# daniestevez/gr4-packet-modem

Hardware: AMD Instinct MI355X
Metric: RX Msamples/s (syncword-detect + RRC chain) (higher is better)
Workload: dtype f32; 1 GPU; configs[1]: 1 channel/GPU, full RX front end (SyncwordDetection 9 bins FFT 2048 + tag gate + CFC + 32-arm RRC SymbolFilter + wipe-off + Costas) on resident burst+AWGN stream; channels_per_gpu=1, freq_bins=9, parallelism=channel-per-gpu x1, input=generated on each GPU, pipelined_streams=4, pipeline_driver=native (gr4pm_packet_receiver), windows=2, correlator_lookahead=2

## Files before the change

### gr4-packet-modem_amd/_abi.py

```python
import ctypes as C
import os

import numpy as np

_HERE = os.path.dirname(os.path.abspath(__file__))
LIB_PATH = os.environ.get("GR4PM_LIB") or os.path.join(_HERE, "libgr4pm_hip.so")

OK = 0
INSUFFICIENT_INPUT_ITEMS = 1
INSUFFICIENT_OUTPUT_ITEMS = 2
TAG_SYNCWORD = 1
TAG_OTHER = 2

TAG_DTYPE = np.dtype(
    [
        ("index", "<u8"),
        ("amplitude", "<f4"),
        ("phase", "<f4"),
        ("freq", "<f8"),
        ("freq_bin", "<i4"),
        ("noise_power", "<f4"),
        ("esn0_db", "<f4"),
        ("time_est", "<f4"),
        ("flags", "<i4"),
# ... 144 lines not shown
                ("pdu_symbols", C.c_void_p), ("n_pdu_symbols", C.c_size_t), ("symbol_pdus", C.c_void_p),
                ("n_symbol_pdus", C.c_size_t), ("symbol_pdu_resyncs", C.c_size_t)]


SYMBOL_PDU_DTYPE = np.dtype([("offset", "<u8"), ("length", "<u8"), ("kind", "<i4"), ("first", "<i4"), ("last", "<i4"),
                             ("pad", "<i4")])
SYMBOL_PDU_FN = C.CFUNCTYPE(None, C.c_void_p, C.c_int, C.c_void_p, C.c_size_t)


class PfbArbParams(C.Structure):
    _fields_ = [("rate", C.c_double), ("rate_is_double", C.c_int), ("taps", C.c_void_p),
                ("n_taps", C.c_size_t), ("filter_size", C.c_size_t), ("stream", C.c_void_p)]


class NoiseSourceParams(C.Structure):
    _fields_ = [("item_kind", C.c_int), ("noise_type", C.c_int), ("amplitude", C.c_float), ("seed", C.c_uint64),
                ("max_items", C.c_size_t), ("stream", C.c_void_p)]


EXPORTS = [
    "gr4pm_last_error", "gr4pm_version", "gr4pm_device_count", "gr4pm_set_deferred_sync", "gr4pm_sincosf", "gr4pm_costas_phase_wrap",
    "gr4pm_packet_receiver_set_symbol_pdu_callback",
    "gr4pm_packet_receiver_publish_symbol_pdus",
    "gr4pm_zmq_pub_create",
    "gr4pm_zmq_pub_destroy",
    "gr4pm_zmq_pub_send",
    "gr4pm_zmq_pub_port",
    "gr4pm_zmq_pub_subscribers",
    "gr4pm_zmq_pub_dropped",
    "gr4pm_syncword_detection_create", "gr4pm_syncword_detection_destroy",
    "gr4pm_syncword_detection_reset", "gr4pm_syncword_detection_syncword_samples_size",
    "gr4pm_syncword_detection_self_corr", "gr4pm_syncword_detection_items_consumed", "gr4pm_syncword_detection_scan_counts",
    "gr4pm_syncword_detection_process", "gr4pm_syncword_detection_last_zpow",
    "gr4pm_syncword_detection_correlate_only",
    "gr4pm_syncword_detection_hint_next", "gr4pm_syncword_detection_announce",
    "gr4pm_syncword_detection_filter_create", "gr4pm_syncword_detection_filter_destroy",
    "gr4pm_syncword_detection_filter_reset", "gr4pm_syncword_detection_filter_process",
    "gr4pm_syncword_detection_filter_gate", "gr4pm_syncword_detection_filter_gate_resolve",
    "gr4pm_payload_metadata_insert_resolve",
    "gr4pm_rotator_create", "gr4pm_rotator_destroy", "gr4pm_rotator_reset", "gr4pm_rotator_process",
    "gr4pm_costas_loop_create", "gr4pm_costas_loop_destroy", "gr4pm_costas_loop_reset",
    "gr4pm_costas_loop_coeffs", "gr4pm_costas_loop_set", "gr4pm_costas_loop_process",
    "gr4pm_syncword_wipeoff_create", "gr4pm_syncword_wipeoff_destroy", "gr4pm_syncword_wipeoff_reset",
    "gr4pm_syncword_wipeoff_process",
    "gr4pm_interp_fir_create", "gr4pm_interp_fir_destroy", "gr4pm_interp_fir_reset",
    "gr4pm_interp_fir_process",
    "gr4pm_symbol_filter_create", "gr4pm_symbol_filter_destroy", "gr4pm_symbol_filter_reset",
    "gr4pm_symbol_filter_process", "gr4pm_cfc_symbol_filter_process",
    "gr4pm_cfc_symbol_filter_plan", "gr4pm_cfc_symbol_filter_run",
    "gr4pm_cfc_symbol_filter_plan_channels", "gr4pm_cfc_symbol_filter_run_channel",
    "gr4pm_cfc_symbol_filter_run_channels", "gr4pm_syncword_wipeoff_process_channels",
    "gr4pm_multichannel_receiver_set_input_in_place", "gr4pm_costas_loop_process_ragged", "gr4pm_costas_loop_set_small_footprint",
    "gr4pm_pfb_arb_resampler_create", "gr4pm_pfb_arb_resampler_destroy", "gr4pm_pfb_arb_resampler_reset",
    "gr4pm_pfb_arb_resampler_process",
    "gr4pm_firdes_root_raised_cosine",
    "gr4pm_payload_metadata_insert_create", "gr4pm_payload_metadata_insert_destroy",
    "gr4pm_payload_metadata_insert_reset", "gr4pm_payload_metadata_insert_process",
    "gr4pm_costas_loop_process_packets",
    "gr4pm_syncword_remove_create", "gr4pm_syncword_remove_destroy", "gr4pm_syncword_remove_reset",
    "gr4pm_syncword_remove_process",
    "gr4pm_constellation_llr_decoder_create", "gr4pm_constellation_llr_decoder_destroy",
    "gr4pm_constellation_llr_decoder_process",
    "gr4pm_additive_scrambler_create", "gr4pm_additive_scrambler_destroy", "gr4pm_additive_scrambler_reset",
    "gr4pm_additive_scrambler_process",
    "gr4pm_header_payload_split_create", "gr4pm_header_payload_split_destroy",
    "gr4pm_header_payload_split_reset", "gr4pm_header_payload_split_process", "gr4pm_header_payload_split_process_c64",
# ... 25 lines not shown
    if _lib is not None:
        return _lib
    if not os.path.exists(LIB_PATH):
        raise ImportError(
            f"{LIB_PATH} is missing: build it with `python -c 'import __graft_entry__ as g; g.build()'` "
            "(hipcc --offload-arch=gfx950). There is no CPU fallback.")
    try:
        import torch
    except ImportError:
        pass
    L = C.CDLL(LIB_PATH)
    vp, sz, szp = C.c_void_p, C.c_size_t, C.POINTER(C.c_size_t)
    L.gr4pm_last_error.restype = C.c_char_p
    L.gr4pm_version.restype = C.c_char_p
    L.gr4pm_device_count.restype = C.c_int
    if hasattr(L, "gr4pm_test_fail_allocations"):
        L.gr4pm_test_fail_allocations.argtypes = [C.c_long, C.c_long]
        L.gr4pm_test_fail_allocations.restype = None
        L.gr4pm_test_allocation_count.restype = C.c_ulonglong
    L.gr4pm_syncword_detection_create.argtypes = [C.POINTER(SyncwordDetectionParams), C.POINTER(vp)]
    L.gr4pm_syncword_detection_destroy.argtypes = [vp]
    L.gr4pm_syncword_detection_destroy.restype = None
    L.gr4pm_syncword_detection_reset.argtypes = [vp]
    L.gr4pm_syncword_detection_syncword_samples_size.argtypes = [vp]
    L.gr4pm_syncword_detection_syncword_samples_size.restype = sz
    L.gr4pm_syncword_detection_self_corr.argtypes = [vp]
    L.gr4pm_syncword_detection_self_corr.restype = C.c_float
    L.gr4pm_syncword_detection_items_consumed.argtypes = [vp]
    L.gr4pm_syncword_detection_items_consumed.restype = C.c_uint64
    L.gr4pm_syncword_detection_scan_counts.argtypes = [vp, sz, C.POINTER(C.c_uint64), C.POINTER(C.c_uint64)]
    L.gr4pm_syncword_detection_scan_counts.restype = None
    L.gr4pm_syncword_detection_process.argtypes = [vp, vp, sz, sz, vp, sz, szp, vp, sz, vp]
    L.gr4pm_syncword_detection_last_zpow.argtypes = [vp, vp, sz]
    L.gr4pm_syncword_detection_correlate_only.argtypes = [vp, vp, sz, sz]
    L.gr4pm_syncword_detection_hint_next.argtypes = [vp, vp, sz, sz]
    L.gr4pm_syncword_detection_announce.argtypes = [vp, vp, sz, sz]
    L.gr4pm_syncword_detection_filter_create.argtypes = [C.POINTER(SdfParams), C.POINTER(vp)]
    L.gr4pm_syncword_detection_filter_destroy.argtypes = [vp]
    L.gr4pm_syncword_detection_filter_destroy.restype = None
    L.gr4pm_syncword_detection_filter_reset.argtypes = [vp]
    L.gr4pm_syncword_detection_filter_process.argtypes = [vp, vp, sz, vp, sz, C.c_int, vp, sz, sz, szp, szp, szp,
                                                          C.POINTER(C.c_int)]
    L.gr4pm_syncword_detection_filter_gate.argtypes = [vp, vp, sz, vp, sz, C.c_int, vp, szp]
    L.gr4pm_rotator_create.argtypes = [C.POINTER(RotatorParams), C.POINTER(vp)]
    L.gr4pm_rotator_destroy.argtypes = [vp]
    L.gr4pm_rotator_destroy.restype = None
    L.gr4pm_rotator_reset.argtypes = [vp]
    L.gr4pm_rotator_process.argtypes = [vp, vp, sz, sz, vp, vp, vp, sz]
    L.gr4pm_costas_loop_create.argtypes = [C.POINTER(CostasParams), C.POINTER(vp)]
    L.gr4pm_costas_loop_destroy.argtypes = [vp]
    L.gr4pm_costas_loop_destroy.restype = None
    L.gr4pm_costas_loop_reset.argtypes = [vp]
    L.gr4pm_costas_loop_coeffs.argtypes = [vp, C.POINTER(C.c_float), C.POINTER(C.c_float)]
    L.gr4pm_costas_loop_coeffs.restype = None
    L.gr4pm_costas_loop_set.argtypes = [vp, C.c_double, C.c_int]
    L.gr4pm_costas_loop_process.argtypes = [vp, vp, sz, sz, vp, vp, vp, sz]
    L.gr4pm_syncword_wipeoff_create.argtypes = [C.POINTER(WipeoffParams), C.POINTER(vp)]
    L.gr4pm_syncword_wipeoff_destroy.argtypes = [vp]
    L.gr4pm_syncword_wipeoff_destroy.restype = None
    L.gr4pm_syncword_wipeoff_reset.argtypes = [vp]
    L.gr4pm_syncword_wipeoff_process.argtypes = [vp, vp, sz, vp, vp, sz]
    L.gr4pm_syncword_wipeoff_process_channels.argtypes = [vp, sz, vp, sz, vp, vp, vp]
    L.gr4pm_cfc_symbol_filter_run_channels.argtypes = [vp, C.c_int, vp, sz, vp, sz, sz, vp, sz, vp, vp, vp, sz, vp, vp, vp, sz, sz]
    L.gr4pm_multichannel_receiver_set_input_in_place.argtypes = [vp, C.c_int]
    L.gr4pm_interp_fir_create.argtypes = [C.POINTER(InterpFirParams), C.POINTER(vp)]
    L.gr4pm_interp_fir_destroy.argtypes = [vp]
# ... 118 lines not shown
```

### gr4-packet-modem_amd/blocks.py

```python
import ctypes as C
import os

import numpy as np

from . import _abi
from ._abi import PACKET_TAG_DTYPE, TAG_DTYPE, TAG_OTHER, TAG_SYNCWORD, Gr4pmError, check, lib

CONSTELLATIONS = {"PILOT": 0, "BPSK": 1, "QPSK": 2}


def _torch():
    import torch
    return torch


def _stream_handle():
    torch = _torch()
    if not torch.cuda.is_available():
        raise Gr4pmError("no HIP device: the gr4pm blocks have no CPU fallback")
    return C.c_void_p(torch.cuda.current_stream().cuda_stream)


def _release(name, h):
    try:
# ... 159 lines not shown
            nx = _dev_c64(next_x)
            nx2 = nx.reshape(1, -1) if nx.dim() == 1 else nx
            assert nx2.shape[0] == self.n_channels
            check(lib().gr4pm_syncword_detection_hint_next(self._h, nx2.data_ptr(), nx2.stride(0), nx2.shape[1]),
                  "SyncwordDetection.hint_next")
        out = torch.empty_like(x2) if want_output else None
        n_done = C.c_size_t(0)
        tags = np.zeros((self.n_channels, tags_cap), dtype=TAG_DTYPE)
        n_tags = (C.c_size_t * self.n_channels)()
        st = lib().gr4pm_syncword_detection_process(
            self._h, x2.data_ptr(), x2.stride(0), n_in, out.data_ptr() if want_output else None,
            out.stride(0) if want_output else 0, C.byref(n_done), _np_ptr(tags), tags_cap, n_tags)
        check(st, "SyncwordDetection.processBulk")
        n = n_done.value
        tag_list = [tags[c, : n_tags[c]].copy() for c in range(self.n_channels)]
        if want_output:
            out = out[:, :n]
            if x.dim() == 1:
                out = out[0]
        if x.dim() == 1:
            tag_list = tag_list[0]
        return st, out, tag_list, n

    def correlate_only(self, x):
        x2 = x.reshape(1, -1) if x.dim() == 1 else x
        check(lib().gr4pm_syncword_detection_correlate_only(self._h, x2.data_ptr(), x2.stride(0), x2.shape[1]),
              "correlate_only")

    def last_zpow(self, n_done):
        torch = _torch()
        z = torch.empty((self.n_channels, n_done), dtype=torch.float32, device="cuda")
        check(lib().gr4pm_syncword_detection_last_zpow(self._h, z.data_ptr(), z.stride(0)), "last_zpow")
        return z

    def _destroy(self):
        if getattr(self, "_h", None):
            _release("gr4pm_syncword_detection_destroy", self._h)
            self._h = None

    def __del__(self):
        try:
            self._destroy()
        except Exception:
            pass


class SyncwordDetectionFilter:

    def __init__(self, samples_per_symbol=4, syncword_size=64, header_size=128):
        self.samples_per_symbol, self.syncword_size, self.header_size = samples_per_symbol, syncword_size, header_size
        p = _abi.SdfParams(samples_per_symbol, syncword_size, header_size, _stream_handle())
        self._h = C.c_void_p()
        check(lib().gr4pm_syncword_detection_filter_create(C.byref(p), C.byref(self._h)), "SyncwordDetectionFilter")

    def start(self):
        check(lib().gr4pm_syncword_detection_filter_reset(self._h), "start")

    def process_bulk(self, x, out, head_tag_flags=0, headers=(), n_ignored=0):
        x = _dev_c64(x)
        msgs = (_abi.HeaderMsg * max(len(headers), 1))()
        for i, hm in enumerate(headers):
            msgs[i].packet_length = 0 if hm is None else hm
            msgs[i].invalid_header = 1 if hm is None else 0
        c, hc, ic, tf = C.c_size_t(0), C.c_size_t(0), C.c_size_t(0), C.c_int(0)
        check(lib().gr4pm_syncword_detection_filter_process(
            self._h, x.data_ptr(), x.numel(), out.data_ptr(), out.numel(), head_tag_flags, msgs, len(headers),
# ... 1558 lines not shown
```

### gr4-packet-modem_amd/csrc/syncword_detection.hip

```cpp
#include <algorithm>
#include <chrono>
#include <cmath>
#include <complex>
#include <cstdint>
#include <deque>
#include <string>
#include <vector>

#include "common.hpp"
#include "fft2048_wave.hpp"
#include "fft2048_pair.hpp"
#include "fft2048_w64.hpp"

#ifndef GR4PM_ABL
#define GR4PM_ABL 0
#endif

namespace gr4pm {

namespace {

constexpr int kWavesPerWg = 4;
constexpr int kMaxBins = 64;
#ifndef GR4PM_TILE_W
#define GR4PM_TILE_W 32768
#endif
constexpr uint32_t kTileW = GR4PM_TILE_W;
constexpr int kAhead = 2, kSets = kAhead + 1, kCarry = kAhead + 2;

struct RawTag {
    uint64_t pos;
    float zx, zy;
    float zpow, left, right, prev, next, noise;
    int32_t bin_idx;
    int32_t pad;
};

__device__ __forceinline__ void wave_lds_sync()
{
    asm volatile("" ::: "memory");
    __builtin_amdgcn_wave_barrier();
    asm volatile("" ::: "memory");
}

__device__ __forceinline__ void fft1_wave(int lane, cf* r, cf* lds, const cf* tw1a, const cf* tw1b)
// ... 502 lines not shown
    }
#pragma unroll
    for (int q = (2 * TQ - 1) / 4 * 4; q < 2 * TQ - 1; ++q) acc += full[q] < thr ? 1u : 0u;
    acc += (at_or_before && prv[R] < thr) ? 1u : 0u;
    acc += (at_or_after && nxt[R] < thr) ? 1u : 0u;
    asm volatile("s_nop 1\n\t"
                 "v_add_u32_dpp %0, %0, %0 row_shr:1 row_mask:0xf bank_mask:0xf bound_ctrl:0\n\t"
                 "s_nop 1\n\t"
                 "v_add_u32_dpp %0, %0, %0 row_shr:2 row_mask:0xf bank_mask:0xf bound_ctrl:0\n\t"
                 "s_nop 1\n\t"
                 "v_add_u32_dpp %0, %0, %0 row_shr:4 row_mask:0xf bank_mask:0xf bound_ctrl:0\n\t"
                 "s_nop 1\n\t"
                 "v_add_u32_dpp %0, %0, %0 row_shr:8 row_mask:0xf bank_mask:0xf bound_ctrl:0\n\t"
                 "s_nop 1\n\t"
                 "v_add_u32_dpp %0, %0, %0 row_bcast:15 row_mask:0xa bank_mask:0xf\n\t"
                 "s_nop 1\n\t"
                 "v_add_u32_dpp %0, %0, %0 row_bcast:31 row_mask:0xc bank_mask:0xf"
                 : "+v"(acc));
    const uint32_t below = static_cast<uint32_t>(__builtin_amdgcn_readlane(static_cast<int>(acc), 63));
    return 2u * below >= 2u * T + 1u;
}
template <int TQ, int R>
__device__ __forceinline__ bool median_dispatch(int r, const float* prv, const float* cur, const float* nxt, int lp, int lane,
                                                float power_threshold)
{
    if constexpr (R >= TQ) {
        return false;
    } else {
        if (r == R) return median_in_registers<TQ, R>(prv, cur, nxt, lp, lane, power_threshold);
        return median_dispatch<TQ, R + 1>(r, prv, cur, nxt, lp, lane, power_threshold);
    }
}

template <int TQ, bool MEDIAN>
__global__ __launch_bounds__(64) void k_candidates_wave(const float* __restrict__ zbase, size_t z_stride, uint32_t cnt,
                                                        uint32_t n_words, uint32_t chain,
                                                        unsigned long long* __restrict__ bitmap, size_t bm_stride,
                                                        unsigned long long* __restrict__ passmap,
                                                        unsigned long long* __restrict__ defermap, float power_threshold)
{
    constexpr uint32_t T = TQ * 64;
    const int lane = threadIdx.x, rl = 63 - lane;
    const float* z = zbase + static_cast<size_t>(blockIdx.y) * z_stride;
    unsigned long long* bmp = bitmap + static_cast<size_t>(blockIdx.y) * bm_stride;
    unsigned long long* pmp = MEDIAN ? passmap + 2 * static_cast<size_t>(blockIdx.y) * bm_stride : nullptr;
    (void)defermap;
    constexpr uint32_t kTestsPerBlock = 8;
    const uint32_t avail = cnt + T;
    const uint32_t n_blk = (n_words + TQ - 1) / TQ;
    const uint32_t b0 = blockIdx.x * chain;
    if (b0 >= n_blk) return;
    const uint32_t b1 = min(b0 + chain, n_blk);
    auto load = [&](uint32_t b, float* v) {
        if ((b + 1) * T <= avail) {
            const char* zb = reinterpret_cast<const char*>(z + static_cast<size_t>(b) * T);
            const uint32_t voff = 4u * static_cast<uint32_t>(rl);
#pragma unroll
            for (int r = 0; r < TQ; ++r)
                v[r] = *reinterpret_cast<const float*>(zb + static_cast<size_t>(voff) + 256 * r);
            return;
        }
#pragma unroll
        for (int r = 0; r < TQ; ++r) {
            const uint32_t g = b * T + 64u * r + rl;
            v[r] = g < avail ? z[g] : -INFINITY;
        }
    };
    auto scans = [&](const float* v, int* rowmax) {
        float t[TQ];
#pragma unroll
        for (int r = 0; r < TQ; ++r) t[r] = v[r];
        if constexpr (TQ % 4 == 0) {
#pragma unroll
            for (int r = 0; r < TQ; r += 4) wave_prefix_max4(t[r], t[r + 1], t[r + 2], t[r + 3]);
        } else {
#pragma unroll
            for (int r = 0; r < TQ; ++r) t[r] = wave_prefix_max(t[r]);
        }
#pragma unroll
        for (int r = 0; r < TQ; ++r) rowmax[r] = fkey(__builtin_amdgcn_readlane(__builtin_bit_cast(int, t[r]), 63));
    };
    const int ninf = fkey(__builtin_bit_cast(int, -INFINITY));
    float cur[TQ], nxt[TQ], prv[MEDIAN ? TQ : 1];
    int rowmax[TQ];
    load(b0, cur);
    if (MEDIAN) {
#pragma unroll
        for (int r = 0; r < TQ; ++r) {
            const long long g = static_cast<long long>(b0) * T - static_cast<long long>(T) + 64 * r + rl;
            prv[r] = g < static_cast<long long>(avail) ? z[g] : -INFINITY;
        }
    }
    scans(cur, rowmax);
    unsigned long long before_mine = 0;
    for (uint32_t b = b0; b < b1; ++b) {
        load(b + 1, nxt);
        int nrowmax[TQ], before[TQ];
        scans(nxt, nrowmax);
        before[0] = ninf;
#pragma unroll
        for (int r = 1; r < TQ; ++r) before[r] = max(before[r - 1], nrowmax[r - 1]);
        unsigned long long mine = 0;
        int after = ninf;
#pragma unroll
        for (int r = TQ - 1; r >= 0; --r) {
            const int U = max(after, before[r]);
            unsigned long long word = 0;
            if (rowmax[r] >= U) {
                const float fwd = __shfl(nxt[r], rl);
                const float pr = __shfl(wave_prefix_max(fwd), rl);
                const float sfx = wave_prefix_max(cur[r]);
                const float m = fmaxf(fmaxf(wave_prev(sfx), __builtin_bit_cast(float, fkey(U))), pr);
                const uint32_t pos = b * T + 64u * r + rl;
                word = __brevll(__ballot(pos < cnt && cur[r] >= m));
            }
            if (lane == r) mine = word;
            after = max(after, rowmax[r]);
        }
        unsigned long long mine_pass = 0, mine_defer = 0;
        if (MEDIAN) {
            unsigned long long rows = __ballot(mine != 0);
            uint32_t tests_left = kTestsPerBlock;
            int prev_pos = -1;
            const bool have_before = b != b0;
            while (rows) {
                const int r = __ffsll(static_cast<long long>(rows)) - 1;
                rows &= rows - 1;
                const unsigned long long word =
                    (static_cast<unsigned long long>(static_cast<uint32_t>(__builtin_amdgcn_readlane(static_cast<int>(mine >> 32), r))) << 32) |
                    static_cast<uint32_t>(__builtin_amdgcn_readlane(static_cast<int>(mine), r));
// ... 9 lines not shown
                    const int o = 64 * r + bit;
                    bool visitable = true;
                    if (prev_pos >= 0) {
                        visitable = false;
                        if (have_before) {
                            const int lo = prev_pos, hi = o - 1, rlo = lo >> 6, rhi = hi >> 6;
                            unsigned long long mask = ~0ull;
                            if (lane == rlo) mask &= ~0ull << (lo & 63);
                            if (lane == rhi) mask &= ~0ull >> (63 - (hi & 63));
                            visitable = __ballot(lane >= rlo && lane <= rhi && (before_mine & mask) != 0) != 0;
                        }
                    }
                    prev_pos = o;
                    if (visitable && tests_left != 0) {
                        --tests_left;
                        if (median_dispatch<TQ, 0>(r, prv, cur, nxt, 63 - bit, lane, power_threshold)) passed |= 1ull << bit;
                    } else {
                        deferred |= 1ull << bit;
                    }
                }
                if (lane == r) {
                    mine_pass = passed;
                    mine_defer = deferred;
                }
            }
            before_mine = mine;
        }
        const uint32_t w = b * TQ + lane;
        if (lane < TQ && w < n_words) {
            bmp[w] = mine;
            if (MEDIAN)
                reinterpret_cast<ulonglong2*>(pmp)[w] = make_ulonglong2(mine_pass, mine_defer);
        }
#pragma unroll
        for (int r = 0; r < TQ; ++r) {
            if (MEDIAN) prv[r] = cur[r];
            cur[r] = nxt[r];
            rowmax[r] = nrowmax[r];
        }
    }
}


__device__ __forceinline__ uint32_t next_candidate(const unsigned long long* bm, uint32_t r, uint32_t hi)
{
    if (r >= hi) return hi;
    uint32_t w = r >> 6;
    unsigned long long word = bm[w] & (~0ull << (r & 63));
    const uint32_t wlast = (hi - 1) >> 6;
    while (true) {
        if (word) {
            const uint32_t p = (w << 6) + static_cast<uint32_t>(__ffsll(static_cast<long long>(word)) - 1);
            return p < hi ? p : hi;
        }
        if (w == wlast) return hi;
        word = bm[++w];
    }
}

constexpr int kTileChunks = static_cast<int>(kTileW / 4096);
static_assert(kTileW % 4096 == 0 && kTileChunks >= 1 && kTileChunks <= 16, "tile = whole 4096-item chunks");
struct TileBits {
    unsigned long long w[kTileChunks];
    uint32_t lo;
    __device__ __forceinline__ void load(const unsigned long long* bm, uint32_t lo_, uint32_t hi, int lane)
    {
        lo = __builtin_amdgcn_readfirstlane(lo_);
        const uint32_t w0 = lo >> 6, wlast = (hi - 1) >> 6;
#pragma unroll
        for (int k = 0; k < kTileChunks; ++k) {
            const uint32_t wi = w0 + 64u * k + lane;
// ... 935 lines not shown
        for (size_t i = 0; i < n; i += len) {
            for (size_t k = 0; k < len / 2; ++k) {
                const double ang = -2.0 * M_PI * static_cast<double>(k) / static_cast<double>(len);
                const std::complex<double> w(std::cos(ang), std::sin(ang));
                const auto u = a[i + k], v = a[i + k + len / 2] * w;
                a[i + k] = u + v;
                a[i + k + len / 2] = u - v;
            }
        }
    }
}

}
}

using namespace gr4pm;

struct gr4pm_syncword_detection {
    size_t fft_size, sps, n_channels, max_items;
    int min_bin, max_bin, n_bins;
    uint64_t T;
    float power_threshold;
    hipStream_t stream;
    size_t L, S, hist;
    float self_corr;
    uint32_t xc, zc;
    size_t z_stride, bm_stride, table_stride;
    uint32_t noise_off = 0;
    uint32_t max_tiles, det_cap, rec_cap;
    DevBuf<float4> tmpl;
    DevBuf<cf> tw;
    bool lds_candidates = false;
    bool separate_median = false;
    bool w64_no_prune = false;
    int corr_kind = 0;
    DevBuf<float4> tmpl64, tT64;
    DevBuf<cf> td;
    DevBuf<cf> cc64;
    int n_cus = 256;
    int w64_variant = -1;
    int w64_one = -1;
    bool coresident = false;
    uint32_t w64_blocks_per_wave = 6;
    PinnedBuf<unsigned> fault;
    int spin_limit = 1 << 20;
    bool use_pair = false;
    DevBuf<float4> tmplp;
    DevBuf<cf> twp;
    bool generic = false;
    int log2n = 0;
    DevBuf<cf> g_tmpl, g_tw;
    DevBuf<cf> tw4k;
    int c4096_variant = 1;
    bool force_radix2 = false;
    DevBuf<cf> carry[kCarry];
    DevBuf<float> z[kSets];
    DevBuf<unsigned long long> bitmap[kSets];
    DevBuf<unsigned long long> passmap[kSets];
    bool fused_median[kSets] = {};
    bool last_fused = false;
    DevBuf<uint32_t> table[kSets];
    DevBuf<unsigned long long> gtable[kSets], gentry, sgtable[kSets];
    size_t gtable_stride = 0, sgtable_stride = 0;
    bool super_level = true;
    uint32_t max_groups = 0;
    DevBuf<int32_t> entry;
// ... 244 lines not shown
    const uint32_t T = static_cast<uint32_t>(h->T);
    const unsigned nch = static_cast<unsigned>(h->n_channels);
    float* zw = h->z[which].p;
    GR4PM_TRY(launch_correlate(h, stream, in, in_stride, n_blocks, zw + h->zc));
    const bool ahead = stream != h->stream;
    static const bool one_front_stream = getenv("GR4PM_SD_FRONT_ONE_STREAM") != nullptr;
    if (ahead && !one_front_stream) {
        GR4PM_HIP_TRY(hipEventRecord(h->ev_mid[which], stream));
        stream = h->stream3;
        GR4PM_HIP_TRY(hipStreamWaitEvent(stream, h->ev_mid[which], 0));
    }
    hipLaunchKernelGGL(k_update_zcarry, dim3((h->zc + 255) / 256, nch), dim3(256), 0, stream,
                       h->z[(which + kSets - 1) % kSets].p, zw, h->z_stride, h->zc, n_prev, h->noise_off,
                       static_cast<uint32_t>(n_prev / h->S));
    hipLaunchKernelGGL(k_update_carry, dim3((h->xc + 255) / 256, nch), dim3(256), 0, stream,
                       reinterpret_cast<const cf*>(in), in_stride, h->carry[ci].p, h->carry[(ci + 1) % kCarry].p,
                       static_cast<size_t>(h->xc), h->xc, J);
    const uint64_t A0 = E0 > T ? E0 - T : 0, A1 = E1 > T ? E1 - T : 0;
    const uint32_t cnt = static_cast<uint32_t>(A1 - A0);
    if (cnt == 0) {
        if (ahead) {
            GR4PM_HIP_TRY(hipEventRecord(h->ev_front[which], stream));
            h->front_recorded[which] = true;
        }
        return GR4PM_OK;
    }
    const float* zloc = zw + h->zc - static_cast<ptrdiff_t>(E0 - A0);
    const uint32_t n_wg = (cnt + kCandTile - 1) / kCandTile;
    const size_t smem = (static_cast<size_t>(kCandBlocks + (T >> 6) + 2) * 65 + kCandBlocks) * sizeof(float);
    h->fused_median[which] = false;
    if (T == 768 && !h->lds_candidates) {
        const uint32_t n_words = n_wg * (kCandTile / 64), n_blk = (n_words + 11) / 12;
        if (!h->separate_median) {
            static const uint32_t kChain = experiment_env_wg("GR4PM_CAND_CHAIN", 8u, 1u, 64u);
            h->fused_median[which] = true;
            hipLaunchKernelGGL((k_candidates_wave<12, true>), dim3((n_blk + kChain - 1) / kChain, nch), dim3(64), 0, stream,
                               zloc, h->z_stride, cnt, n_words, kChain, h->bitmap[which].p, h->bm_stride,
                               h->passmap[which].p, nullptr, h->power_threshold);
        } else {
            constexpr uint32_t kChain = 8;
            hipLaunchKernelGGL((k_candidates_wave<12, false>), dim3((n_blk + kChain - 1) / kChain, nch), dim3(64), 0, stream,
                               zloc, h->z_stride, cnt, n_words, kChain, h->bitmap[which].p, h->bm_stride, nullptr, nullptr, 0.0f);
        }
    } else {
        hipLaunchKernelGGL(k_candidates, dim3(n_wg, nch), dim3(256), smem, stream, zloc, h->z_stride, cnt, T,
                           h->bitmap[which].p, h->bm_stride);
    }
    const uint32_t n_tiles = (cnt + kTileW - 1) / kTileW;
    hipLaunchKernelGGL(k_tile_tables, dim3(n_tiles, nch), dim3(64), 0, stream, h->bitmap[which].p, h->bm_stride,
                       cnt, T, n_tiles, h->table[which].p, h->table_stride);
    const uint32_t n_groups = (n_tiles + kGroup - 1) / kGroup;
    hipLaunchKernelGGL(k_group_tables, dim3((T + 1 + 127) / 128, n_groups, nch), dim3(128), 0, stream, cnt, T,
                       n_tiles, h->table[which].p, h->table_stride, h->gtable[which].p, h->gtable_stride);
    if (h->super_level && n_groups > kSuper)
        hipLaunchKernelGGL(k_super_tables, dim3((T + 1 + 127) / 128, (n_groups + kSuper - 1) / kSuper, nch), dim3(128), 0,
                           stream, cnt, T, n_tiles, n_groups, h->gtable[which].p, h->gtable_stride, h->sgtable[which].p,
                           h->sgtable_stride);
    GR4PM_HIP_TRY(hipGetLastError());
    if (ahead) {
        GR4PM_HIP_TRY(hipEventRecord(h->ev_front[which], stream));
        h->front_recorded[which] = true;
    }
    return GR4PM_OK;
}

gr4pm_status ensure_ahead_streams(gr4pm_syncword_detection* h)
{
    if (h->stream2) return GR4PM_OK;
    int least = 0, greatest = 0;
// ... 178 lines not shown
        const char* one = getenv("GR4PM_W64_ONE");
        h->w64_one = one ? atoi(one) : -1;
        if (h->w64_one > 1 && !experiment_env("GR4PM_W64_ONE", true)) h->w64_one = 1;
        if (const char* b = getenv("GR4PM_W64_BLOCKS_PER_WAVE")) h->w64_blocks_per_wave = static_cast<uint32_t>(std::max(0, atoi(b)));
        int dev = 0;
        hipDeviceProp_t prop;
        if (hipGetDevice(&dev) == hipSuccess && hipGetDeviceProperties(&prop, dev) == hipSuccess)
            h->n_cus = prop.multiProcessorCount;
        if (const char* c = getenv("GR4PM_W64_CUS")) h->n_cus = std::max(1, std::min(h->n_cus, atoi(c)));
    }

    h->xc = static_cast<uint32_t>(round_up(h->hist + h->S + 2, 64));
    h->zc = static_cast<uint32_t>(round_up(2 * h->T + 2, 64));
    h->noise_off = static_cast<uint32_t>(h->zc + round_up(h->max_items, 64) + 64);
    h->z_stride = h->noise_off + round_up(h->max_items / h->S + 4, 64);
    const size_t max_cnt = h->max_items + h->T;
    h->bm_stride = round_up(max_cnt, kCandTile) / 64 + 16;
    h->max_tiles = static_cast<uint32_t>((max_cnt + kTileW - 1) / kTileW);
    h->table_stride = static_cast<size_t>(h->max_tiles) * (h->T + 1);
    h->det_cap = static_cast<uint32_t>(h->max_items / (h->T + 1) + 16);
    h->rec_cap = h->det_cap;
    gr4pm_status s = GR4PM_OK;
    auto ok = [&](gr4pm_status r) {
        if (s == GR4PM_OK) s = r;
    };
    ok(h->tmpl.alloc(tmpl.size()));
    ok(h->tw.alloc(tw.size()));
    ok(h->tmplp.alloc(tmplp.size()));
    ok(h->fault.alloc(1));
    if (h->fault.p) *h->fault.p = 0;
    if (const char* e = getenv("GR4PM_TEST_SPIN_LIMIT")) h->spin_limit = atoi(e);
    h->lds_candidates = getenv("GR4PM_CANDIDATES_LDS") != nullptr;
    h->separate_median = getenv("GR4PM_SD_SEPARATE_MEDIAN") != nullptr;
    h->w64_no_prune = getenv("GR4PM_W64_NO_PRUNE") != nullptr;
    ok(h->tmpl64.alloc(tmpl64.size()));
    ok(h->tT64.alloc(tT64.size()));
    ok(h->td.alloc(td.size()));
    ok(h->cc64.alloc(cc64.size()));
    ok(h->twp.alloc(twp.size()));
    std::vector<cf> g_tw(h->generic ? p->fft_size / 2 : 0);
    for (size_t k = 0; k < g_tw.size(); ++k) {
        const double ang = -2.0 * M_PI * static_cast<double>(k) / static_cast<double>(p->fft_size);
        g_tw[k] = mk(static_cast<float>(std::cos(ang)), static_cast<float>(std::sin(ang)));
    }
    std::vector<cf> tw4k(16 * 256 + 256);
    if (h->generic && p->fft_size == static_cast<size_t>(kN4k)) {
        build_4096_tables(
            [](int k) {
                const double ang = -2.0 * M_PI * k / kN4k;
                return mk(static_cast<float>(std::cos(ang)), static_cast<float>(std::sin(ang)));
            },
            tw4k.data(), tw4k.data() + 16 * 256);
        ok(h->tw4k.alloc(tw4k.size()));
        const char* e = getenv("GR4PM_CORRELATOR");
        h->force_radix2 = e && std::string(e) == "radix2";
    }
    if (h->generic) {
        ok(h->g_tmpl.alloc(g_tmpl.size()));
        ok(h->g_tw.alloc(g_tw.size()));
        const int lds_bytes = static_cast<int>(2 * p->fft_size * sizeof(cf)) + 2048;
        if (hipFuncSetAttribute(reinterpret_cast<const void*>(k_correlate_generic),
                                hipFuncAttributeMaxDynamicSharedMemorySize, lds_bytes) != hipSuccess ||
            hipFuncSetAttribute(reinterpret_cast<const void*>(k_tags_generic),
                                hipFuncAttributeMaxDynamicSharedMemorySize, lds_bytes) != hipSuccess) {
            set_error("cannot reserve %d bytes of LDS for fft_size %zu", lds_bytes, p->fft_size);
            ok(GR4PM_ERR_HIP);
// ... 132 lines not shown
    static double t_acc[4] = { 0, 0, 0, 0 };
    static int t_calls = 0;
    const auto tp0 = std::chrono::steady_clock::now();
#endif
    const uint32_t n_blocks = static_cast<uint32_t>((n_in - h->fft_size) / h->S + 1);
    const size_t J = static_cast<size_t>(n_blocks) * h->S;
    const uint64_t E0 = h->items_consumed, E1 = E0 + J;
    const uint32_t T = static_cast<uint32_t>(h->T);
    const int cur = (h->cur + 1) % kSets;
    const unsigned nch = static_cast<unsigned>(h->n_channels);
    hipStream_t s = h->stream;
    float* zcur = h->z[cur].p;
    const cf* carry = h->carry[h->ci].p;

    bool have_front = false;
    if (!h->launched.empty()) {
        const auto& a = h->launched.front();
        if (a.in == in && a.stride == in_stride && a.n == n_in && a.E0 == E0 && a.set == cur) {
            GR4PM_HIP_TRY(hipStreamWaitEvent(s, h->ev_front[cur], 0));
            h->launched.pop_front();
            have_front = true;
        } else {
            for (const auto& l : h->launched) GR4PM_HIP_TRY(hipStreamWaitEvent(s, h->ev_front[l.set], 0));
            h->launched.clear();
        }
    }
    if (!have_front) GR4PM_TRY(launch_front(h, s, cur, h->ci, in, in_stride, n_in, E0, h->last_done));
    const bool order_by_event = !have_front && !h->announced.empty();
    if (order_by_event) GR4PM_HIP_TRY(hipEventRecord(h->ev_zcarry, s));

    const uint64_t A0 = E0 > T ? E0 - T : 0, A1 = E1 > T ? E1 - T : 0;
    const uint32_t cnt = static_cast<uint32_t>(A1 - A0);
    const float* zloc = zcur + h->zc - static_cast<ptrdiff_t>(E0 - A0);
    if (cnt > 0) {
        const uint32_t n_tiles = (cnt + kTileW - 1) / kTileW;
        const uint32_t n_groups = (n_tiles + kGroup - 1) / kGroup;
        hipLaunchKernelGGL(k_scan_entries, dim3(nch), dim3(256), 0, s, h->st.p, static_cast<unsigned long long>(A0),
                           cnt, T, n_tiles, h->table[cur].p, h->table_stride, h->gtable[cur].p, h->gtable_stride,
                           h->gentry.p, n_groups, h->entry.p,
                           h->super_level && n_groups > kSuper ? h->sgtable[cur].p : nullptr, h->sgtable_stride);
        hipLaunchKernelGGL(k_tile_visit, dim3((n_tiles + kVisitWaves - 1) / kVisitWaves, nch), dim3(64 * kVisitWaves), 0, s,
                           h->bitmap[cur].p, h->bm_stride, cnt, T,
                           n_tiles, h->entry.p, h->st.p, h->visit.p, h->visit_cap);
        const uint32_t n_vis = cnt / (T + 1) + n_tiles + 1;
        const uint32_t median_grid = std::max<uint32_t>(64u, 16384u / nch);
        h->last_fused = h->fused_median[cur];
        if (h->fused_median[cur]) {
            hipLaunchKernelGGL(k_resolve_visited, dim3((n_vis + 256 * kResolveWaves - 1) / (256 * kResolveWaves), nch),
                               dim3(64 * kResolveWaves), 0, s,
                               static_cast<unsigned long long>(A0), h->st.p, h->visit.p, h->visit_cap, h->passmap[cur].p,
                               h->bm_stride, h->det.p, h->det_cap, h->deferred.p);
            hipLaunchKernelGGL(k_median_tests<true>, dim3(std::min<uint32_t>(n_vis, median_grid), nch), dim3(64), 0, s, zloc,
                               h->z_stride, static_cast<unsigned long long>(A0), T, h->power_threshold, h->st.p,
                               h->deferred.p, h->visit_cap, h->det.p, h->det_cap);
        } else {
            hipLaunchKernelGGL(k_median_tests<false>, dim3(std::min<uint32_t>(n_vis, median_grid), nch), dim3(64), 0, s, zloc,
                               h->z_stride, static_cast<unsigned long long>(A0), T, h->power_threshold, h->st.p, h->visit.p,
                               h->visit_cap, h->det.p, h->det_cap);
        }
    }
    if (h->generic && h->fft_size == static_cast<size_t>(kN4k) && !h->force_radix2 && h->hist <= h->S) {
        hipLaunchKernelGGL((k_tags<false, 9>), dim3(std::min<uint32_t>(h->det_cap, 4096u) / kTagWaves<false>, nch),
                           dim3(64 * kTagWaves<false>), 0, s,
                           reinterpret_cast<const cf*>(in), in_stride, carry, static_cast<size_t>(h->xc), h->xc,
                           static_cast<unsigned long long>(E0), static_cast<unsigned long long>(E1),
                           static_cast<uint32_t>(h->hist), static_cast<uint32_t>(h->S), h->n_bins, h->tmpl.p, h->tw.p, h->tw.p,
// ... 122 lines not shown
    }
    if (ret == GR4PM_ERR_OVERFLOW) set_error("tags_cap too small");
#ifdef GR4PM_TIMING
    {
        const auto tp4 = std::chrono::steady_clock::now();
        auto us = [](auto a, auto b) { return std::chrono::duration<double, std::micro>(b - a).count(); };
        t_acc[0] += us(tp0, tp1);
        t_acc[1] += us(tp1, tp2);
        t_acc[2] += us(tp2, tp3);
        t_acc[3] += us(tp3, tp4);
        if (++t_calls % 8 == 0) {
            fprintf(stderr, "[gr4pm timing] launch %.0f us, sync %.0f us, records %.0f us, finish %.0f us (mean of the last 8)\n",
                    t_acc[0] / 8, t_acc[1] / 8, t_acc[2] / 8, t_acc[3] / 8);
            t_acc[0] = t_acc[1] = t_acc[2] = t_acc[3] = 0;
        }
    }
#endif
    return ret;
}
GR4PM_ABI_CATCH

gr4pm_status gr4pm_syncword_detection_last_zpow(gr4pm_syncword_detection* h, float* zpow, size_t stride)
try {
    if (!h || !zpow) return GR4PM_ERR_INVALID;
    for (size_t c = 0; c < h->n_channels; ++c) {
        GR4PM_HIP_TRY(hipMemcpyAsync(zpow + c * stride, h->z[h->cur].p + c * h->z_stride + h->zc,
                                     h->last_done * sizeof(float), hipMemcpyDeviceToDevice, h->stream));
    }
    GR4PM_HIP_TRY(hipStreamSynchronize(h->stream));
    return GR4PM_OK;
}
GR4PM_ABI_CATCH

}
```

### include/gr4pm_hip.h

```cpp
#ifndef GR4PM_HIP_H
#define GR4PM_HIP_H

#include <stddef.h>
#include <stdint.h>

#ifdef __cplusplus
extern "C" {
#endif

typedef struct { float re, im; } gr4pm_c64;

typedef enum {
    GR4PM_OK = 0,
    GR4PM_INSUFFICIENT_INPUT_ITEMS = 1,
    GR4PM_INSUFFICIENT_OUTPUT_ITEMS = 2,
    GR4PM_ERR_INVALID = -1,
    GR4PM_ERR_UNSUPPORTED = -2,
    GR4PM_ERR_HIP = -3,
    GR4PM_ERR_NOMEM = -4,
    GR4PM_ERR_OVERFLOW = -5,
    GR4PM_ERR_NO_DEVICE = -6,
    GR4PM_ERR_INTERNAL = -7
} gr4pm_status;

// ... 30 lines not shown
    size_t n_syncword;
    const gr4pm_c64* constellation;
    size_t n_constellation;
    int min_freq_bin;
    int max_freq_bin;
    uint64_t time_threshold;
    float power_threshold;
    size_t n_channels;
    size_t max_items;
    void* stream;
} gr4pm_syncword_detection_params;

gr4pm_status gr4pm_syncword_detection_create(const gr4pm_syncword_detection_params* params,
                                             gr4pm_syncword_detection** out);
void gr4pm_syncword_detection_destroy(gr4pm_syncword_detection* h);
gr4pm_status gr4pm_syncword_detection_reset(gr4pm_syncword_detection* h);
size_t gr4pm_syncword_detection_syncword_samples_size(const gr4pm_syncword_detection* h);
float gr4pm_syncword_detection_self_corr(const gr4pm_syncword_detection* h);
uint64_t gr4pm_syncword_detection_items_consumed(const gr4pm_syncword_detection* h);
void gr4pm_syncword_detection_scan_counts(const gr4pm_syncword_detection* h, size_t channel, uint64_t* visited,
                                          uint64_t* tested_from_memory);
gr4pm_status gr4pm_syncword_detection_process(gr4pm_syncword_detection* h, const gr4pm_c64* in,
                                              size_t in_stride, size_t n_in, gr4pm_c64* out,
                                              size_t out_stride, size_t* n_done, gr4pm_tag* tags,
                                              size_t tags_cap, size_t* n_tags);
#define GR4PM_SD_LOOKAHEAD 2
gr4pm_status gr4pm_syncword_detection_announce(gr4pm_syncword_detection* h, const gr4pm_c64* in,
                                               size_t in_stride, size_t n_in);
gr4pm_status gr4pm_syncword_detection_hint_next(gr4pm_syncword_detection* h,
                                                const gr4pm_c64* in_next, size_t in_stride,
                                                size_t n_next);
gr4pm_status gr4pm_syncword_detection_last_zpow(gr4pm_syncword_detection* h, float* zpow,
                                                size_t stride);
gr4pm_status gr4pm_syncword_detection_correlate_only(gr4pm_syncword_detection* h,
                                                     const gr4pm_c64* in, size_t in_stride,
                                                     size_t n_in);

typedef struct gr4pm_syncword_detection_filter gr4pm_syncword_detection_filter;
typedef struct {
    size_t samples_per_symbol;
    size_t syncword_size;
    size_t header_size;
    void* stream;
} gr4pm_syncword_detection_filter_params;
typedef struct {
    uint64_t packet_length;
    int32_t invalid_header;
} gr4pm_header_msg;
gr4pm_status gr4pm_syncword_detection_filter_create(
    const gr4pm_syncword_detection_filter_params* params, gr4pm_syncword_detection_filter** out);
void gr4pm_syncword_detection_filter_destroy(gr4pm_syncword_detection_filter* h);
gr4pm_status gr4pm_syncword_detection_filter_reset(gr4pm_syncword_detection_filter* h);
gr4pm_status gr4pm_syncword_detection_filter_process(
    gr4pm_syncword_detection_filter* h, const gr4pm_c64* in, size_t n_in, gr4pm_c64* out,
    size_t out_cap, int head_tag_flags, const gr4pm_header_msg* headers, size_t n_headers,
    size_t n_ignored, size_t* consumed, size_t* headers_consumed, size_t* ignored_consumed,
    int* tag_out_flags);

gr4pm_status gr4pm_syncword_detection_filter_gate(gr4pm_syncword_detection_filter* h,
                                                  const uint64_t* tag_index, size_t n_tags,
                                                  const gr4pm_header_msg* headers, size_t n_headers,
                                                  int headers_per_tag, uint8_t* accepted,
                                                  size_t* headers_used);
gr4pm_status gr4pm_syncword_detection_filter_gate_resolve(gr4pm_syncword_detection_filter* h,
                                                          const gr4pm_header_msg* msg);

// ... 462 lines not shown
```

Baseline: 66430 Msamples/s.

## Transpose candidate row-max with permlane swaps and rotate buffers in candidate kernel

Rewrites the per-row max reduction in the fused candidate kernel. Rows are folded pairwise with v_permlane32/16_swap and v_max before DPP row_shr reductions, so fewer registers need the full-wave scan. The block loop also rotates three register buffers through a 3x manual unroll instead of copying cur/nxt/prv each iteration. A debug export for reading back candidate bitmaps is added. The risks are extra register pressure from the three buffers and correctness hazards in the inline asm lane layout.

```diff
diff --git a/gr4-packet-modem_amd/_abi.py b/gr4-packet-modem_amd/_abi.py
--- a/gr4-packet-modem_amd/_abi.py
+++ b/gr4-packet-modem_amd/_abi.py
@@ -200,6 +200,7 @@
     "gr4pm_syncword_detection_reset", "gr4pm_syncword_detection_syncword_samples_size",
     "gr4pm_syncword_detection_self_corr", "gr4pm_syncword_detection_items_consumed", "gr4pm_syncword_detection_scan_counts",
     "gr4pm_syncword_detection_process", "gr4pm_syncword_detection_last_zpow",
+    "gr4pm_syncword_detection_last_candidate_words",
     "gr4pm_syncword_detection_correlate_only",
     "gr4pm_syncword_detection_hint_next", "gr4pm_syncword_detection_announce",
     "gr4pm_syncword_detection_filter_create", "gr4pm_syncword_detection_filter_destroy",
@@ -291,6 +292,8 @@
     L.gr4pm_syncword_detection_scan_counts.restype = None
     L.gr4pm_syncword_detection_process.argtypes = [vp, vp, sz, sz, vp, sz, szp, vp, sz, vp]
     L.gr4pm_syncword_detection_last_zpow.argtypes = [vp, vp, sz]
+    if hasattr(L, "gr4pm_syncword_detection_last_candidate_words"):
+        L.gr4pm_syncword_detection_last_candidate_words.argtypes = [vp, vp, vp, sz, C.POINTER(sz)]
     L.gr4pm_syncword_detection_correlate_only.argtypes = [vp, vp, sz, sz]
     L.gr4pm_syncword_detection_hint_next.argtypes = [vp, vp, sz, sz]
     L.gr4pm_syncword_detection_announce.argtypes = [vp, vp, sz, sz]
diff --git a/gr4-packet-modem_amd/blocks.py b/gr4-packet-modem_amd/blocks.py
--- a/gr4-packet-modem_amd/blocks.py
+++ b/gr4-packet-modem_amd/blocks.py
@@ -215,6 +215,15 @@
         z = torch.empty((self.n_channels, n_done), dtype=torch.float32, device="cuda")
         check(lib().gr4pm_syncword_detection_last_zpow(self._h, z.data_ptr(), z.stride(0)), "last_zpow")
         return z
+
+    def last_candidate_words(self):
+        n = C.c_size_t(0)
+        cap = self.max_items // 64 + 128
+        bm = np.zeros((self.n_channels, cap), dtype=np.uint64)
+        pd = np.zeros((self.n_channels, cap, 2), dtype=np.uint64)
+        check(lib().gr4pm_syncword_detection_last_candidate_words(self._h, _np_ptr(bm), _np_ptr(pd), cap, C.byref(n)),
+              "last_candidate_words")
+        return bm[:, :n.value].copy(), pd[:, :n.value].copy()
 
     def _destroy(self):
         if getattr(self, "_h", None):
diff --git a/gr4-packet-modem_amd/csrc/candidates_rowmax.hpp b/gr4-packet-modem_amd/csrc/candidates_rowmax.hpp
--- /dev/null
+++ b/gr4-packet-modem_amd/csrc/candidates_rowmax.hpp
@@ -0,0 +1,151 @@
+#pragma once
+#include <math.h>
+
+#include "fft2048_wave.hpp"
+
+namespace gr4pm {
+
+template <int TQ>
+struct RowMaxLayout {
+    static constexpr int P = (TQ + 3) / 4 * 4, H = P / 2, Q = P / 4;
+    static constexpr int reg(int r) { return r % Q; }
+    static constexpr int lane(int r) { return 16 * (r / Q) + 15; }
+};
+
+template <int TQ, class Ops, class V>
+GR4PM_HD void rowmax_transposed(V* v, V* d)
+{
+    using L = RowMaxLayout<TQ>;
+    V pad[L::P - TQ + 1];
+    for (int k = 0; k < L::P - TQ; ++k) pad[k] = Ops::splat(-INFINITY);
+    V c[L::H];
+#if defined(__clang__)
+#pragma unroll
+#endif
+    for (int k = 0; k < L::H; k += 2) {
+        V& a0 = v[k];
+        V& a1 = v[k + 1];
+        V& b0 = k + L::H < TQ ? v[k + L::H] : pad[k + L::H < TQ ? 0 : k + L::H - TQ];
+        V& b1 = k + 1 + L::H < TQ ? v[k + 1 + L::H] : pad[k + 1 + L::H < TQ ? 0 : k + 1 + L::H - TQ];
+        Ops::fold32x2(a0, b0, a1, b1, c[k], c[k + 1]);
+    }
+#if defined(__clang__)
+#pragma unroll
+#endif
+    for (int k = 0; k < L::Q; ++k) Ops::fold16(c[k], c[k + L::Q], d[k]);
+    Ops::template row_reduce<L::Q>(d);
+}
+
+struct RowMaxHostWave {
+    float l[64];
+};
+struct RowMaxHostOps {
+    using V = RowMaxHostWave;
+    static V splat(float x)
+    {
+        V v;
+        for (float& e : v.l) e = x;
+        return v;
+    }
+    static void swap32(V& a, V& b)
+    {
+        for (int i = 0; i < 32; ++i) {
+            const float t = a.l[32 + i];
+            a.l[32 + i] = b.l[i];
+            b.l[i] = t;
+        }
+    }
+    static void swap16(V& a, V& b)
+    {
+        for (int row = 0; row < 4; row += 2)
+            for (int i = 0; i < 16; ++i) {
+                const float t = a.l[16 * (row + 1) + i];
+                a.l[16 * (row + 1) + i] = b.l[16 * row + i];
+                b.l[16 * row + i] = t;
+            }
+    }
+    static V vmax(const V& a, const V& b)
+    {
+        V m;
+        for (int i = 0; i < 64; ++i) m.l[i] = fmaxf(a.l[i], b.l[i]);
+        return m;
+    }
+    static void max_row_shr(V& a, int n)
+    {
+        const V old = a;
+        for (int i = 0; i < 64; ++i)
+            if (i % 16 >= n) a.l[i] = fmaxf(old.l[i - n], old.l[i]);
+    }
+    static void fold32x2(V& a0, V& b0, V& a1, V& b1, V& m0, V& m1)
+    {
+        swap32(a0, b0);
+        swap32(a1, b1);
+        m0 = vmax(a0, b0);
+        m1 = vmax(a1, b1);
+        swap32(a0, b0);
+        swap32(a1, b1);
+    }
+    static void fold16(V& a, V& b, V& m)
+    {
+        swap16(a, b);
+        m = vmax(a, b);
+    }
+    template <int N>
+    static void row_reduce(V* d)
+    {
+        for (int n = 1; n < 16; n *= 2)
+            for (int k = 0; k < N; ++k) max_row_shr(d[k], n);
+    }
+};
+
+#if defined(__HIPCC__)
+struct RowMaxDeviceOps {
+    static __device__ __forceinline__ float splat(float x) { return x; }
+    static __device__ __forceinline__ void fold32x2(float& a0, float& b0, float& a1, float& b1, float& m0, float& m1)
+    {
+        asm volatile("s_nop 1\n\t"
+                     "v_permlane32_swap_b32 %0, %1\n\t"
+                     "v_permlane32_swap_b32 %2, %3\n\t"
+                     "v_max_f32 %4, %0, %1\n\t"
+                     "v_max_f32 %5, %2, %3\n\t"
+                     "v_permlane32_swap_b32 %0, %1\n\t"
+                     "v_permlane32_swap_b32 %2, %3"
+                     : "+v"(a0), "+v"(b0), "+v"(a1), "+v"(b1), "=&v"(m0), "=&v"(m1));
+    }
+    static __device__ __forceinline__ void fold16(float& a, float& b, float& m)
+    {
+        asm volatile("s_nop 1\n\t"
+                     "v_permlane16_swap_b32 %0, %1\n\t"
+                     "v_max_f32 %2, %0, %1"
+                     : "+v"(a), "+v"(b), "=&v"(m));
+    }
+    template <int N>
+    static __device__ __forceinline__ void row_reduce(float* d)
+    {
+        if constexpr (N == 3) {
+#define GR4PM_STEP(ctl)                                    \
+    "v_max_f32_dpp %0, %0, %0 " ctl "\n\t"                 \
+    "v_max_f32_dpp %1, %1, %1 " ctl "\n\t"                 \
+    "v_max_f32_dpp %2, %2, %2 " ctl "\n\t"
+            asm volatile("s_nop 1\n\t" GR4PM_STEP("row_shr:1 row_mask:0xf bank_mask:0xf") GR4PM_STEP("row_shr:2 row_mask:0xf bank_mask:0xf")
+                             GR4PM_STEP("row_shr:4 row_mask:0xf bank_mask:0xf") GR4PM_STEP("row_shr:8 row_mask:0xf bank_mask:0xf")
+                         : "+v"(d[0]), "+v"(d[1]), "+v"(d[2]));
+#undef GR4PM_STEP
+        } else {
+#pragma unroll
+            for (int k = 0; k < N; ++k)
+                asm volatile("s_nop 1\n\t"
+                             "v_max_f32_dpp %0, %0, %0 row_shr:1 row_mask:0xf bank_mask:0xf\n\t"
+                             "s_nop 1\n\t"
+                             "v_max_f32_dpp %0, %0, %0 row_shr:2 row_mask:0xf bank_mask:0xf\n\t"
+                             "s_nop 1\n\t"
+                             "v_max_f32_dpp %0, %0, %0 row_shr:4 row_mask:0xf bank_mask:0xf\n\t"
+                             "s_nop 1\n\t"
+                             "v_max_f32_dpp %0, %0, %0 row_shr:8 row_mask:0xf bank_mask:0xf"
+                             : "+v"(d[k]));
+        }
+    }
+};
+#endif
+
+}
diff --git a/gr4-packet-modem_amd/csrc/syncword_detection.hip b/gr4-packet-modem_amd/csrc/syncword_detection.hip
--- a/gr4-packet-modem_amd/csrc/syncword_detection.hip
+++ b/gr4-packet-modem_amd/csrc/syncword_detection.hip
@@ -11,6 +11,7 @@
 #include "fft2048_wave.hpp"
 #include "fft2048_pair.hpp"
 #include "fft2048_w64.hpp"
+#include "candidates_rowmax.hpp"
 
 #ifndef GR4PM_ABL
 #define GR4PM_ABL 0
@@ -579,7 +580,7 @@
     }
 }
 
-template <int TQ, bool MEDIAN>
+template <int TQ, bool MEDIAN, int FORM = 0>
 __global__ __launch_bounds__(64) void k_candidates_wave(const float* __restrict__ zbase, size_t z_stride, uint32_t cnt,
                                                         uint32_t n_words, uint32_t chain,
                                                         unsigned long long* __restrict__ bitmap, size_t bm_stride,
@@ -613,7 +614,16 @@
             v[r] = g < avail ? z[g] : -INFINITY;
         }
     };
-    auto scans = [&](const float* v, int* rowmax) {
+    auto scans = [&](float* v, int* rowmax) {
+        if constexpr (FORM >= 1) {
+            using L = RowMaxLayout<TQ>;
+            float d[L::Q];
+            rowmax_transposed<TQ, RowMaxDeviceOps>(v, d);
+#pragma unroll
+            for (int r = 0; r < TQ; ++r)
+                rowmax[r] = fkey(__builtin_amdgcn_readlane(__builtin_bit_cast(int, d[L::reg(r)]), L::lane(r)));
+            return;
+        }
         float t[TQ];
 #pragma unroll
         for (int r = 0; r < TQ; ++r) t[r] = v[r];
@@ -628,8 +638,10 @@
         for (int r = 0; r < TQ; ++r) rowmax[r] = fkey(__builtin_amdgcn_readlane(__builtin_bit_cast(int, t[r]), 63));
     };
     const int ninf = fkey(__builtin_bit_cast(int, -INFINITY));
-    float cur[TQ], nxt[TQ], prv[MEDIAN ? TQ : 1];
-    int rowmax[TQ];
+    float buf[3][TQ];
+    int rmax[3][TQ];
+    float *const prv = buf[0], *const cur = buf[1];
+    int* const rowmax = rmax[1];
     load(b0, cur);
     if (MEDIAN) {
 #pragma unroll
@@ -640,9 +652,10 @@
     }
     scans(cur, rowmax);
     unsigned long long before_mine = 0;
-    for (uint32_t b = b0; b < b1; ++b) {
+    auto block = [&](uint32_t b, const float* prv, const float* cur, float* nxt, const int* rowmax, int* nrowmax)
+                     __attribute__((always_inline)) {
         load(b + 1, nxt);
-        int nrowmax[TQ], before[TQ];
+        int before[TQ];
         scans(nxt, nrowmax);
         before[0] = ninf;
 #pragma unroll
@@ -718,11 +731,27 @@
             if (MEDIAN)
                 reinterpret_cast<ulonglong2*>(pmp)[w] = make_ulonglong2(mine_pass, mine_defer);
         }
-#pragma unroll
-        for (int r = 0; r < TQ; ++r) {
-            if (MEDIAN) prv[r] = cur[r];
-            cur[r] = nxt[r];
-            rowmax[r] = nrowmax[r];
+    };
+    if constexpr (FORM >= 2) {
+        for (uint32_t b = b0;;) {
+            block(b, buf[0], buf[1], buf[2], rmax[1], rmax[2]);
+            if (++b >= b1) break;
+            block(b, buf[1], buf[2], buf[0], rmax[2], rmax[0]);
+            if (++b >= b1) break;
+            block(b, buf[2], buf[0], buf[1], rmax[0], rmax[1]);
+            if (++b >= b1) break;
+        }
+    } else {
+        float* const nxt = buf[2];
+        int* const nrowmax = rmax[2];
+        for (uint32_t b = b0; b < b1; ++b) {
+            block(b, prv, cur, nxt, rowmax, nrowmax);
+#pragma unroll
+            for (int r = 0; r < TQ; ++r) {
+                if (MEDIAN) prv[r] = cur[r];
+                cur[r] = nxt[r];
+                rowmax[r] = nrowmax[r];
+            }
         }
     }
 }
@@ -1724,6 +1753,9 @@
     DevBuf<cf> tw;
     bool lds_candidates = false;
     bool separate_median = false;
+    uint32_t cand_form = 2;
+    uint32_t cand_chain = 8;
+    uint32_t last_cand_cnt = 0;
     bool w64_no_prune = false;
     int corr_kind = 0;
     DevBuf<float4> tmpl64, tT64;
@@ -2034,9 +2066,12 @@
     if (T == 768 && !h->lds_candidates) {
         const uint32_t n_words = n_wg * (kCandTile / 64), n_blk = (n_words + 11) / 12;
         if (!h->separate_median) {
-            static const uint32_t kChain = experiment_env_wg("GR4PM_CAND_CHAIN", 8u, 1u, 64u);
+            const uint32_t kChain = h->cand_chain;
             h->fused_median[which] = true;
-            hipLaunchKernelGGL((k_candidates_wave<12, true>), dim3((n_blk + kChain - 1) / kChain, nch), dim3(64), 0, stream,
+            auto kernel = h->cand_form == 0   ? k_candidates_wave<12, true, 0>
+                          : h->cand_form == 1 ? k_candidates_wave<12, true, 1>
+                                              : k_candidates_wave<12, true, 2>;
+            hipLaunchKernelGGL(kernel, dim3((n_blk + kChain - 1) / kChain, nch), dim3(64), 0, stream,
                                zloc, h->z_stride, cnt, n_words, kChain, h->bitmap[which].p, h->bm_stride,
                                h->passmap[which].p, nullptr, h->power_threshold);
         } else {
@@ -2281,6 +2316,8 @@
     if (const char* e = getenv("GR4PM_TEST_SPIN_LIMIT")) h->spin_limit = atoi(e);
     h->lds_candidates = getenv("GR4PM_CANDIDATES_LDS") != nullptr;
     h->separate_median = getenv("GR4PM_SD_SEPARATE_MEDIAN") != nullptr;
+    h->cand_form = experiment_env_wg("GR4PM_CAND_FORM", 2u, 0u, 2u);
+    h->cand_chain = experiment_env_wg("GR4PM_CAND_CHAIN", 8u, 1u, 64u);
     h->w64_no_prune = getenv("GR4PM_W64_NO_PRUNE") != nullptr;
     ok(h->tmpl64.alloc(tmpl64.size()));
     ok(h->tT64.alloc(tT64.size()));
@@ -2479,6 +2516,7 @@
     const uint64_t A0 = E0 > T ? E0 - T : 0, A1 = E1 > T ? E1 - T : 0;
     const uint32_t cnt = static_cast<uint32_t>(A1 - A0);
     const float* zloc = zcur + h->zc - static_cast<ptrdiff_t>(E0 - A0);
+    h->last_cand_cnt = cnt;
     if (cnt > 0) {
         const uint32_t n_tiles = (cnt + kTileW - 1) / kTileW;
         const uint32_t n_groups = (n_tiles + kGroup - 1) / kGroup;
@@ -2667,4 +2705,29 @@
 }
 GR4PM_ABI_CATCH
 
-}
+gr4pm_status gr4pm_syncword_detection_last_candidate_words(gr4pm_syncword_detection* h, uint64_t* bitmap,
+                                                           uint64_t* pass_defer, size_t cap, size_t* n_words)
+try {
+    if (!h || !bitmap || !pass_defer || !n_words) return GR4PM_ERR_INVALID;
+    if (!h->last_fused) {
+        set_error("last_candidate_words: the last call did not run the fused candidate kernel");
+        return GR4PM_ERR_INVALID;
+    }
+    const size_t n = static_cast<size_t>((h->last_cand_cnt + kCandTile - 1) / kCandTile) * (kCandTile / 64);
+    *n_words = n;
+    if (n > cap) {
+        set_error("last_candidate_words: %zu words per channel, room for %zu", n, cap);
+        return GR4PM_ERR_OVERFLOW;
+    }
+    for (size_t c = 0; c < h->n_channels && n; ++c) {
+        GR4PM_HIP_TRY(hipMemcpyAsync(bitmap + c * cap, h->bitmap[h->cur].p + c * h->bm_stride, n * sizeof(uint64_t),
+                                     hipMemcpyDeviceToHost, h->stream));
+        GR4PM_HIP_TRY(hipMemcpyAsync(pass_defer + 2 * c * cap, h->passmap[h->cur].p + 2 * c * h->bm_stride,
+                                     2 * n * sizeof(uint64_t), hipMemcpyDeviceToHost, h->stream));
+    }
+    GR4PM_HIP_TRY(hipStreamSynchronize(h->stream));
+    return GR4PM_OK;
+}
+GR4PM_ABI_CATCH
+
+}
diff --git a/include/gr4pm_hip.h b/include/gr4pm_hip.h
--- a/include/gr4pm_hip.h
+++ b/include/gr4pm_hip.h
@@ -86,6 +86,8 @@
                                                 size_t n_next);
 gr4pm_status gr4pm_syncword_detection_last_zpow(gr4pm_syncword_detection* h, float* zpow,
                                                 size_t stride);
+gr4pm_status gr4pm_syncword_detection_last_candidate_words(gr4pm_syncword_detection* h, uint64_t* bitmap,
+                                                           uint64_t* pass_defer, size_t cap, size_t* n_words);
 gr4pm_status gr4pm_syncword_detection_correlate_only(gr4pm_syncword_detection* h,
                                                      const gr4pm_c64* in, size_t in_stride,
                                                      size_t n_in);
```

Result: no change. 65850 Msamples/s (-0.9%).
